# ttwang0303/Adaptive-RGBD-Localization-Mappig

Hardware: AMD Instinct MI355X
Metric: frames/sec (extract+match+RANSAC-PnP) @640x480, 2000 kp (higher is better)
Workload: dtype u8/i32 (extract, match), f32+f64 (ransac, pnp)

## Files before the change

### adaptive-rgbd-localization-mappig_amd/csrc/k_extract.hip

```cpp
#include "odo_device.h"
#include "odo_internal.h"
#ifdef FS_STATS
#include <cstdio>
#endif

#ifndef ODO_EXTRACT_PRIO
#define ODO_EXTRACT_PRIO 0
#endif
#define EXTRACT_PRIO() \
    if (ODO_EXTRACT_PRIO) __builtin_amdgcn_s_setprio(ODO_EXTRACT_PRIO)

namespace odo {

__global__ void __launch_bounds__(256) k_gray(const uint8_t* __restrict__ bgr, uint8_t* __restrict__ pyr,
                                              int w, int h, int pitch, size_t in_stride, size_t pyr_stride) {
    EXTRACT_PRIO();
    const int f = blockIdx.y;
    const int q = blockIdx.x * blockDim.x + threadIdx.x;
    const uint8_t* src = bgr + (size_t)f * in_stride;
    uint8_t* dst = pyr + (size_t)f * pyr_stride;
    const int npix = w * h;
    const int p0 = q * 4;
    if (p0 >= npix) return;
    const int y = p0 / w, x = p0 - y * w;
// ... 131 lines not shown
    const LevelDesc L = lv[G.level];
    const int R = G.rows, cols = G.cols, BW = G.bw, wcell = G.wcell, nc = G.ncell;
    constexpr int RS = FS_RS, RS4 = RS >> 2;
    const int sh = G.x0 & 15;
    {
        const uint4* src = reinterpret_cast<const uint4*>(pyr + (size_t)f * pyr_stride + L.off +
                                                          (size_t)G.y0 * L.pitch + (G.x0 & ~15));
        const int nw = (sh + cols + 15) >> 4, p16 = L.pitch >> 4;
        const int rstep = FS_TH / nw, k = t % nw, r0 = t / nw;
        if (r0 < rstep)
            for (int r = r0; r < R; r += rstep)
                reinterpret_cast<uint4*>(roi + r * RS)[k] = src[__umul24((uint32_t)r, (uint32_t)p16) + (uint32_t)k];
        for (int i = t; i < (R * RS) >> 4; i += FS_TH) reinterpret_cast<uint4*>(score)[i] = uint4{0, 0, 0, 0};
        for (int i = t; i < R * BW; i += FS_TH) bits[i] = 0;
        for (int i = t; i < R * FS_NCM; i += FS_TH) cnt[i] = 0;
        if (t == 0) M.ncl = 0, M.ovf = 0;
    }
    const int drows = R - 6;
    const int m0 = (sh + 3) >> 2, m1 = (sh + cols - 4) >> 2;
    {
        const uint32_t mlo = (0xFu << (sh + 3 - 4 * m0)) & 0xFu, mhi = (1u << (sh + cols - 3 - 4 * m1)) - 1u;
        if (t <= m1 - m0) {
            const int m = m0 + t;
            qlist[t] = uint2{fs_msb_mask((t == 0 ? mlo : 0xFu) & (m == m1 ? mhi : 0xFu)), 4u * (uint32_t)m};
        }
    }
    __syncthreads();
    const float inv_w = 1.0f / (float)wcell;
    uint32_t* const out = cand + ((size_t)f * ncells + G.ci0) * cell_cap;
    typedef short s16x2 __attribute__((ext_vector_type(2)));
    for (int pass = 0; pass < 2; pass++) {
        const int th = pass == 0 ? ini_th : min_th;
        const int thc = th < 0 ? 0 : (th > 255 ? 255 : th);
        const int NL = pass == 0 ? m1 - m0 + 1 : M.nl;
        const int items = drows > 0 && cols > 6 && NL > 0 ? drows * NL : 0;
        if (t == 0) FS_STAT(pass, items);
        {
            const s16x2 thv = {(short)thc, (short)thc};
            const float inl = NL > 0 ? 1.0f / (float)NL : 0.0f, inl_h = 0.5f * inl;
            int head = 0, tail = 0;
            auto seg_test = [&](int h, int n) {
                const int i0 = 2 * lane, i1 = i0 + 1;
                bool c0 = false, c1 = false;
                int o0 = 0, o1 = 0;
                if (i0 < n) {
                    o0 = ring[(h + i0) & (FS_RING - 1)];
                    o1 = i1 < n ? ring[(h + i1) & (FS_RING - 1)] : o0;
                    const s16x2 vv = {(short)roi[o0], (short)roi[o1]};
                    int a0 = o0 - 3 * RS - 3, a1 = o1 - 3 * RS - 3;
                    asm("" : "+v"(a0), "+v"(a1));
                    const uint8_t* const q0 = roi + a0;
                    const uint8_t* const q1 = roi + a1;
                    s16x2 d[16];
#pragma unroll
                    for (int k = 0; k < 16; k++) {
                        const int off = (kCircleDy[k] + 3) * RS + kCircleDx[k] + 3;
                        s16x2 c;
                        c.x = (short)q0[off];
                        c.y = (short)q1[off];
                        d[k] = vv - c;
                    }
                    s16x2 mn2[8], mx2[8], mn4[8], mx4[8];
#pragma unroll
                    for (int q = 0; q < 8; q++) {
                        const int j = 2 * q + 1;
                        mn2[q] = __builtin_elementwise_min(d[j], d[(j + 1) & 15]);
                        mx2[q] = __builtin_elementwise_max(d[j], d[(j + 1) & 15]);
                    }
#pragma unroll
                    for (int q = 0; q < 8; q++) {
                        mn4[q] = __builtin_elementwise_min(mn2[q], mn2[(q + 1) & 7]);
                        mx4[q] = __builtin_elementwise_max(mx2[q], mx2[(q + 1) & 7]);
                    }
                    s16x2 dk = s16x2{-32768, -32768}, br = s16x2{32767, 32767};
#pragma unroll
                    for (int q = 0; q < 8; q++) {
                        const int k = 2 * q;
                        const s16x2 m8 = __builtin_elementwise_min(mn4[q], mn4[(q + 2) & 7]);
                        const s16x2 x8 = __builtin_elementwise_max(mx4[q], mx4[(q + 2) & 7]);
                        dk = __builtin_elementwise_max(
                            dk, __builtin_elementwise_min(m8, __builtin_elementwise_max(d[k], d[(k + 9) & 15])));
                        br = __builtin_elementwise_min(
                            br, __builtin_elementwise_max(x8, __builtin_elementwise_min(d[k], d[(k + 9) & 15])));
                    }
                    const s16x2 sc = __builtin_elementwise_max(dk, -br);
                    c0 = sc.x > thc;
                    c1 = i1 < n && sc.y > thc;
                    if (c0) score[o0] = (uint8_t)(sc.x - 1);
                    if (c1) score[o1] = (uint8_t)(sc.y - 1);
                }
                const uint64_t b0 = __ballot(c0), b1 = __ballot(c1);
                const int nco = __popcll(b0) + __popcll(b1);
                if (lane == 0) FS_STAT(3, 1);
                if (nco) {
                    int cb = 0;
                    if (lane == 0) cb = atomicAdd(&M.ncl, nco);
                    cb = __shfl(cb, 0);
                    const int pre = (int)__builtin_amdgcn_mbcnt_hi((uint32_t)(b0 >> 32), __builtin_amdgcn_mbcnt_lo((uint32_t)b0, 0)) +
                                    (int)__builtin_amdgcn_mbcnt_hi((uint32_t)(b1 >> 32), __builtin_amdgcn_mbcnt_lo((uint32_t)b1, 0));
                    const int p0 = cb + pre, p1 = p0 + (c0 ? 1 : 0);
                    if (c0) { if (p0 < FS_CL) clist[p0] = (uint16_t)o0; else M.ovf = 1; }
                    if (c1) { if (p1 < FS_CL) clist[p1] = (uint16_t)o1; else M.ovf = 1; }
                }
            };
            for (int base = wave * 64; base < items; base += FS_TH) {
                uint32_t pass4 = 0;
                int qoff = 0;
                const int it = base + lane;
                if (it < items) {
                    const int ii = (int)__builtin_fmaf((float)it, inl, inl_h);
                    const int kk = it - __mul24(ii, NL);
                    const uint2 e = qlist[kk];
                    int wb = (int)__umul24((uint32_t)ii, (uint32_t)RS) + (int)e.y;
                    asm("" : "+v"(wb));
                    qoff = wb + 3 * RS;
                    const uint32_t* w = reinterpret_cast<const uint32_t*>(roi + wb);
                    const uint32_t Cw = w[3 * RS4], Uw = w[0], Dw = w[6 * RS4];
                    const uint32_t Lw = __builtin_amdgcn_alignbyte(Cw, w[3 * RS4 - 1], 1);
                    const uint32_t Rw = __builtin_amdgcn_alignbyte(w[3 * RS4 + 1], Cw, 3);
                    uint32_t hm[2];
#pragma unroll
                    for (int hh = 0; hh < 2; hh++) {
                        const uint32_t sel = hh ? 0x0c030c02u : 0x0c010c00u;
                        s16x2 v, a0, a4, a8, a12;
                        *reinterpret_cast<uint32_t*>(&v) = __builtin_amdgcn_perm(0u, Cw, sel);
                        *reinterpret_cast<uint32_t*>(&a0) = __builtin_amdgcn_perm(0u, Dw, sel);
                        *reinterpret_cast<uint32_t*>(&a4) = __builtin_amdgcn_perm(0u, Rw, sel);
                        *reinterpret_cast<uint32_t*>(&a8) = __builtin_amdgcn_perm(0u, Uw, sel);
                        *reinterpret_cast<uint32_t*>(&a12) = __builtin_amdgcn_perm(0u, Lw, sel);
                        const s16x2 dk = __builtin_elementwise_max(__builtin_elementwise_min(a0, a8),
                                                                   __builtin_elementwise_min(a4, a12));
                        const s16x2 bk = __builtin_elementwise_min(__builtin_elementwise_max(a0, a8),
                                                                   __builtin_elementwise_max(a4, a12));
                        const s16x2 t1 = dk - (v - thv), t2 = (v + thv) - bk;
                        hm[hh] = *reinterpret_cast<const uint32_t*>(&t1) | *reinterpret_cast<const uint32_t*>(&t2);
                    }
                    pass4 = __builtin_amdgcn_perm(hm[1], hm[0], 0x07050301u) & e.x;
                }
                uint32_t pos = (uint32_t)tail;
#pragma unroll
                for (int k = 0; k < 4; k++) {
                    const bool sv = (pass4 >> (8 * k + 7)) & 1u;
                    const uint64_t bk = __ballot(sv);
                    const uint32_t slot =
                        __builtin_amdgcn_mbcnt_hi((uint32_t)(bk >> 32), __builtin_amdgcn_mbcnt_lo((uint32_t)bk, pos)) &
                        (FS_RING - 1);
                    uint32_t at;
                    asm("v_cndmask_b32_e64 %0, %1, %2, %3" : "=v"(at) : "v"((uint32_t)FS_RING), "v"(slot), "s"(bk));
                    ring[at] = (uint16_t)(qoff + k);
                    pos += (uint32_t)__popcll(bk);
                }
                tail = (int)pos;
                if (tail - head >= 128) {
                    wave_lds_sync();
                    do {
                        seg_test(head, 128);
                        head += 128;
                    } while (tail - head >= 128);
                    wave_lds_sync();
                }
            }
            if (lane == 0) FS_STAT(2, tail);
            if (tail > head) {
                wave_lds_sync();
                seg_test(head, tail - head);
            }
        }
        __syncthreads();
        const bool ovf = M.ovf != 0;
        const int ncl = min(M.ncl, FS_CL);
        if (t == 0) FS_STAT(4, M.ncl), FS_STAT(5, ovf ? 1 : 0);
        auto locate = [&](int o, int& r, int& xs, int& jl, int& xl, int& xh) {
            r = o / RS;
            xs = (o - r * RS) - sh;
            jl = (int)(((float)(xs - 3) + 0.5f) * inv_w);
            xl = 3 + jl * wcell;
            xh = min(xl + wcell, cols - 3);
        };
        auto nms = [&](int o) {
            int so = o - RS - 1;
            asm("" : "+v"(so));
            const uint8_t* const sb = score + so;
            const int sc = sb[RS + 1];
            int r, xs, jl, xl, xh;
            locate(o, r, xs, jl, xl, xh);
            const int nmid = max((int)sb[1], (int)sb[2 * RS + 1]);
            const int nl = max(max((int)sb[0], (int)sb[RS]), (int)sb[2 * RS]);
            const int nr = max(max((int)sb[2], (int)sb[RS + 2]), (int)sb[2 * RS + 2]);
            const int nb = max(nmid, max(xs - 1 >= xl ? nl : 0, xs + 1 < xh ? nr : 0));
            if (sc > nb) {
                atomicOr(&bits[r * BW + (xs >> 5)], 1u << (xs & 31));
                atomicAdd(&cnt[r * FS_NCM + jl], 1);
            }
        };
        auto scan = [&](auto&& fn) {
            for (int it = t; it < items; it += FS_TH) {
                const int ii2 = it / NL, kk2 = it - ii2 * NL;
                const uint2 e = qlist[kk2];
                const uint32_t msk = e.x;
                const int qo = (3 + ii2) * RS + (int)e.y;
                for (int b = 0; b < 4; b++)
                    if (((msk >> (8 * b + 7)) & 1u) && score[qo + b]) fn(qo + b);
            }
        };
        if (!ovf)
            for (int i = t; i < ncl; i += FS_TH) nms(clist[i]);
        else
            scan(nms);
        __syncthreads();
        for (int j = wave; j < nc; j += FS_TH / 64) {
            if (pass == 1 && !M.retry[j]) continue;
            const int r = 3 + lane;
            const int v = lane < drows ? cnt[r * FS_NCM + j] : 0;
            int incl = v;
#pragma unroll
            for (int o = 1; o < 64; o <<= 1) {
                const int y = __shfl_up(incl, o);
                if (lane >= o) incl += y;
            }
            if (lane < drows) cnt[r * FS_NCM + j] = incl - v;
            if (lane == 63) M.tot[j] = incl;
        }
        __syncthreads();
        auto place = [&](int o) {
            int r, xs, jl, xl, xh;
            locate(o, r, xs, jl, xl, xh);
            const uint32_t* row = bits + r * BW;
            if (!((row[xs >> 5] >> (xs & 31)) & 1u)) return;
            int rank = cnt[r * FS_NCM + jl];
            const int wl = xl >> 5, nwd = (xs >> 5) - wl;
            const uint32_t hm = (1u << (xs & 31)) - 1u;
#pragma unroll
            for (int i = 0; i < 4; i++) {
                uint32_t v = row[wl + i];
                if (i == 0) v &= ~0u << (xl & 31);
                v &= i < nwd ? ~0u : (i == nwd ? hm : 0u);
                rank += __builtin_popcount(v);
            }
            if (rank < cell_cap)
                out[(size_t)jl * cell_cap + rank] = ((uint32_t)score[o] << 24) |
                                                    ((uint32_t)(r + G.y0 - 16) << 12) | (uint32_t)(xs + G.x0 - 16);
        };
        if (!ovf)
            for (int i = t; i < ncl; i += FS_TH) place(clist[i]);
        else
            scan(place);
        if (pass == 0) {
            if (t < nc) M.retry[t] = M.tot[t] == 0;
            __syncthreads();
            if (t < nc && M.retry[t]) FS_STAT(6, 1);
            if (t == 0) FS_STAT(7, nc);
            if (t < nc) {
                const int xa = sh + 3 + t * wcell, xe = sh + min(3 + (t + 1) * wcell, cols - 3);
                if (M.retry[t]) {
                    int at = 0;
                    for (int j = 0; j < t; j++)
                        if (M.retry[j]) {
                            const int ja = sh + 3 + j * wcell, je = sh + min(3 + (j + 1) * wcell, cols - 3);
                            at += ((je - 1) >> 2) - (ja >> 2) + 1;
                        }
                    for (int m = xa >> 2; m <= (xe - 1) >> 2; m++) {
                        const int lo = max(xa - 4 * m, 0), hi = min(xe - 4 * m, 4);
                        qlist[at++] = uint2{fs_msb_mask((0xFu << lo) & ((1u << hi) - 1u)), 4u * (uint32_t)m};
                    }
                } else {
                    cand_cnt[(size_t)f * ncells + G.ci0 + t] = min(M.tot[t], cell_cap);
                }
            }
            if (t == 0) {
                int n = 0;
                for (int j = 0; j < nc; j++)
                    if (M.retry[j]) {
                        const int ja = sh + 3 + j * wcell, je = sh + min(3 + (j + 1) * wcell, cols - 3);
                        n += ((je - 1) >> 2) - (ja >> 2) + 1;
                    }
                M.nl = n;
                M.ncl = 0;
                M.ovf = 0;
            }
            __syncthreads();
            if (M.nl == 0) return;
        } else if (t < nc && M.retry[t]) {
            cand_cnt[(size_t)f * ncells + G.ci0 + t] = min(M.tot[t], cell_cap);
        }
    }
}

struct ONode {
    int16_t x0, y0, x1, y1;
    int32_t cnt;
    int32_t seq;
};

#ifndef OT_THREADS
#define OT_THREADS 256
#endif

#ifndef OT_KB
#define OT_KB 8
#endif
#ifndef OT_RANK_MAX
#define OT_RANK_MAX 512
#endif
enum { OT_LDK = 1, OT_LDN = 2 };
template <bool RES, int LD, typename F>
ODO_INLINE void ot_pass(int n, int t, uint32_t (&rk)[OT_KB], int (&rn)[OT_KB], const uint32_t* keys, int32_t* knode,
                        F&& f) {
    if constexpr (RES) {
#pragma unroll
        for (int u = 0; u < OT_KB; u++)
            if (t + u * OT_THREADS < n) f(t + u * OT_THREADS, rk[u], rn[u]);
    } else {
        for (int k0 = t; k0 < n; k0 += OT_THREADS * OT_KB) {
#pragma unroll
            for (int u = 0; u < OT_KB; u++) {
                const int k = k0 + u * OT_THREADS;
                rn[u] = -1;
                if (k < n) {
                    if (LD & OT_LDK) rk[u] = keys[k];
                    if (LD & OT_LDN) rn[u] = knode[k];
                }
            }
#pragma unroll
            for (int u = 0; u < OT_KB; u++) {
                const int k = k0 + u * OT_THREADS;
                if (k < n) {
                    int node = rn[u];
                    f(k, rk[u], node);
                    if (node != rn[u]) knode[k] = node;
                }
            }
        }
    }
}

ODO_INLINE int block_exclusive_scan(int v, int* tmp, int* total);

ODO_INLINE int ot_gather(const uint32_t* __restrict__ cand, const int* __restrict__ cand_cnt, size_t cell0, int nc,
                         int cell_cap, uint32_t* dst, int cap, int* scan) {
    const int t = threadIdx.x;
    int n = 0;
    for (int cb = 0; cb < nc; cb += OT_THREADS) {
        const int c = cb + t;
        const int cnt = c < nc ? cand_cnt[cell0 + c] : 0;
        int tot;
        const int ex = block_exclusive_scan(cnt, scan, &tot);
        if (c < nc) {
            const uint4* src = reinterpret_cast<const uint4*>(cand + (cell0 + c) * cell_cap);
            uint32_t* d = dst + n + ex;
            const int room = cap - (n + ex);
            const int m = cnt < room ? cnt : room;
            for (int k0 = 0; k0 < m; k0 += 32) {
                uint4 v[8];
#pragma unroll
                for (int u = 0; u < 8; u++)
                    if (k0 + 4 * u < m) v[u] = src[(k0 >> 2) + u];
#pragma unroll
                for (int u = 0; u < 8; u++) {
                    const int k = k0 + 4 * u;
                    if (k < m) d[k] = v[u].x;
                    if (k + 1 < m) d[k + 1] = v[u].y;
                    if (k + 2 < m) d[k + 2] = v[u].z;
                    if (k + 3 < m) d[k + 3] = v[u].w;
                }
            }
        }
        n += tot;
    }
    return n;
}

ODO_INLINE uint64_t ot_key(int cnt, int seq, int pos) {
    return ((uint64_t)(uint32_t)cnt << 40) | ((uint64_t)(uint32_t)(seq & 0xFFFFFF) << 16) | (uint64_t)(pos & 0xFFFF);
}

ODO_INLINE int block_exclusive_scan(int v, int* tmp, int* total) {
    const int t = threadIdx.x, lane = t & 63, wave = t >> 6;
    const int x = wave_incl_scan(v);
    if (lane == 63) tmp[wave] = x;
    __syncthreads();
    int base = 0, tot = 0;
#pragma unroll
    for (int w = 0; w < OT_THREADS / 64; w++) {
        const int sw = tmp[w];
        if (w < wave) base += sw;
        tot += sw;
    }
    *total = tot;
    __syncthreads();
    return base + x - v;
}
ODO_INLINE int2 block_exclusive_scan2(int a, int b, int* tmp, int2* total) {
    constexpr int NWV = OT_THREADS / 64;
    const int t = threadIdx.x, lane = t & 63, wave = t >> 6;
    const int xa = wave_incl_scan(a), xb = wave_incl_scan(b);
    if (lane == 63) tmp[wave] = xa, tmp[NWV + wave] = xb;
    __syncthreads();
    int ba = 0, bb = 0, ta = 0, tb = 0;
#pragma unroll
    for (int w = 0; w < NWV; w++) {
        const int sa = tmp[w], sb = tmp[NWV + w];
        if (w < wave) ba += sa, bb += sb;
        ta += sa;
        tb += sb;
    }
    *total = int2{ta, tb};
    __syncthreads();
    return int2{ba + xa - a, bb + xb - b};
}

template <bool RES>
ODO_INLINE void ot_tree(const int n, const LevelDesc& L, char* smem, int* s_vars, const int node_cap,
                        uint32_t (&rk)[OT_KB], int (&rn)[OT_KB], const uint32_t* keys, int32_t* knode,
                        uint32_t* __restrict__ out, int* __restrict__ ocnt_fl, const int cap) {
    const int t = threadIdx.x;
    ONode* nodesA = reinterpret_cast<ONode*>(smem);
    ONode* nodesB = nodesA + node_cap;
    int* cc = reinterpret_cast<int*>(nodesB + node_cap);
    int* npos = cc + 4 * node_cap;
    int* iscr = npos + 4 * node_cap;
    int* scan = iscr + node_cap;
    uint64_t* sortk = reinterpret_cast<uint64_t*>(scan + OT_THREADS + 2);
    int& s_J = s_vars[6];
    int& s_size = s_vars[0];
    int& s_prev = s_vars[1];
    int& s_seq = s_vars[2];
    int& s_phase = s_vars[3];
    int& s_finish = s_vars[4];
    int& s_vcnt = s_vars[5];

    const int minX = 16, maxX = L.w - 16, minY = 16, maxY = L.h - 16;
    const int N = L.quota;
    const int nIni = (int)roundf((float)(maxX - minX) / (float)(maxY - minY));
    const float hX = (float)(maxX - minX) / (float)nIni;

    for (int i = t; i < nIni; i += OT_THREADS) {
        ONode nd;
        nd.x0 = (int16_t)(int)(hX * (float)i);
        nd.x1 = (int16_t)(int)(hX * (float)(i + 1));
        nd.y0 = 0;
        nd.y1 = (int16_t)(maxY - minY);
        nd.cnt = 0;
        nd.seq = i;
        nodesA[i] = nd;
    }
    __syncthreads();
    int ic0 = 0, ic1 = 0, ic2 = 0, ic3 = 0;
    ot_pass<RES, OT_LDK>(
        n, t, rk, rn, keys, knode, [&](int k, uint32_t key, int& node) {
            const float x = (float)(key & 0xfff);
            const int ni = (int)(x / hX);
            node = ni;
            ic0 += ni == 0;
            ic1 += ni == 1;
            ic2 += ni == 2;
            ic3 += ni == 3;
            if (ni > 3) atomicAdd(&nodesA[ni].cnt, 1);
        });
    if (ic0) atomicAdd(&nodesA[0].cnt, ic0);
    if (ic1) atomicAdd(&nodesA[1].cnt, ic1);
    if (ic2) atomicAdd(&nodesA[2].cnt, ic2);
    if (ic3) atomicAdd(&nodesA[3].cnt, ic3);
    __syncthreads();
    if (t == 0) {
        int w = 0;
        for (int i = 0; i < nIni; i++) {
            iscr[i] = -1;
            if (nodesA[i].cnt > 0) {
                iscr[i] = w;
                nodesB[w++] = nodesA[i];
            }
        }
        s_size = w;
        s_seq = nIni;
        s_finish = 0;
        s_phase = 1;
    }
    __syncthreads();
    ot_pass<RES, OT_LDN>(n, t, rk, rn, keys, knode, [&](int k, uint32_t key, int& node) { node = iscr[node]; });
    for (int i = t; i < s_size; i += OT_THREADS) nodesA[i] = nodesB[i];
    __syncthreads();

    ONode* cur = nodesA;
    ONode* nxt = nodesB;
    int vcount = 0;

    while (!s_finish) {
        const int S = s_size;
        if (s_phase == 1) {
            for (int i = t; i < 4 * S; i += OT_THREADS) cc[i] = 0;
            __syncthreads();
            ot_pass<RES, OT_LDK | OT_LDN>(
                n, t, rk, rn, keys, knode, [&](int k, uint32_t key, int& node) {
                    const ONode N0 = cur[node];
                    if (N0.cnt > 1) {
                        const int x = key & 0xfff, y = (key >> 12) & 0xfff;
                        const int hx = (N0.x1 - N0.x0 + 1) >> 1;
                        const int hy = (N0.y1 - N0.y0 + 1) >> 1;
                        const int q = (x < N0.x0 + hx) ? (y < N0.y0 + hy ? 0 : 2) : (y < N0.y0 + hy ? 1 : 3);
                        atomicAdd(&cc[node * 4 + q], 1);
                        node |= q << 16;
                    }
                });
            __syncthreads();
            int childBase = 0, survBase = 0, expBase = 0;
            int totalChildren = 0;
            for (int cb = 0; cb < S; cb += OT_THREADS) {
                const int i = cb + t;
                int e = 0, ne = 0, s = 0;
                if (i < S) {
                    if (cur[i].cnt > 1) {
#pragma unroll
                        for (int q = 0; q < 4; q++) {
                            e += cc[i * 4 + q] > 0;
                            ne += cc[i * 4 + q] > 1;
                        }
                    } else s = 1;
                }
                int2 tp;
                const int2 ex = block_exclusive_scan2(e | (ne << 16), s, scan, &tp);
                const int ex_e = ex.x & 0xFFFF, ex_ne = ex.x >> 16, ex_s = ex.y;
                const int te = tp.x & 0xFFFF, tne = tp.x >> 16, ts = tp.y;
                if (i < S) {
                    iscr[i] = childBase + ex_e;
                    npos[i * 4 + 0] = e;
                    npos[i * 4 + 1] = ex_ne + expBase;
                    npos[i * 4 + 2] = survBase + ex_s;
                    npos[i * 4 + 3] = s;
                }
                childBase += te;
                expBase += tne;
                survBase += ts;
                __syncthreads();
            }
            totalChildren = childBase;
            const int newSize = totalChildren + survBase;
            for (int i = t; i < S; i += OT_THREADS) {
                const ONode P = cur[i];
                const int e = npos[i * 4 + 0];
                const int vb = npos[i * 4 + 1];
                const int sr = npos[i * 4 + 2];
                if (npos[i * 4 + 3]) {
                    const int pos = totalChildren + sr;
                    nxt[pos] = P;
                    cc[i * 4 + 0] = pos;
                } else {
                    const int blockStart = totalChildren - (iscr[i] + e);
                    const int hx = (P.x1 - P.x0 + 1) >> 1, hy = (P.y1 - P.y0 + 1) >> 1;
                    int r = 0, v = vb;
                    int cpos[4];
#pragma unroll
                    for (int q = 0; q < 4; q++) {
                        const int c = cc[i * 4 + q];
                        cpos[q] = -1;
                        if (c > 0) {
                            ONode C;
                            const int qx = q & 1, qy = q >> 1;
                            C.x0 = (int16_t)(qx ? P.x0 + hx : P.x0);
                            C.x1 = (int16_t)(qx ? P.x1 : P.x0 + hx);
                            C.y0 = (int16_t)(qy ? P.y0 + hy : P.y0);
                            C.y1 = (int16_t)(qy ? P.y1 : P.y0 + hy);
                            C.cnt = c;
                            C.seq = s_seq + iscr[i] + r;
                            const int pos = blockStart + (e - 1 - r);
                            nxt[pos] = C;
                            cpos[q] = pos;
                            if (c > 1) {
                                sortk[v] = ot_key(c, C.seq, pos);
                                v++;
                            }
                            r++;
                        }
                    }
#pragma unroll
                    for (int q = 0; q < 4; q++) cc[i * 4 + q] = cpos[q];
                }
            }
            __syncthreads();
            ot_pass<RES, OT_LDN>(n, t, rk, rn, keys, knode, [&](int k, uint32_t key, int& node) {
                node = cc[(node & 0xFFFF) * 4 + (node >> 16)];
            });
            if (t == 0) {
                s_prev = S;
                s_size = newSize;
                s_seq += totalChildren;
                s_vcnt = expBase;
                if (newSize >= N || newSize == S) s_finish = 1;
                else if (newSize + expBase * 3 > N) s_phase = 2;
            }
            vcount = expBase;
            ONode* tmpp = cur;
            cur = nxt;
            nxt = tmpp;
        } else {
            vcount = s_vcnt;
            for (int i = t; i < S; i += OT_THREADS) iscr[i] = -1;
            if (vcount <= OT_RANK_MAX) {
                __syncthreads();
                for (int i = t; i < vcount; i += OT_THREADS) {
                    const uint64_t ki = sortk[i];
                    int above = 0, j = 0;
                    for (; j + 8 <= vcount; j += 8) {
                        uint64_t kj[8];
#pragma unroll
                        for (int u = 0; u < 8; u++) kj[u] = sortk[j + u];
#pragma unroll
                        for (int u = 0; u < 8; u++) above += kj[u] > ki;
                    }
                    for (; j < vcount; j++) above += sortk[j] > ki;
                    iscr[(int)(ki & 0xFFFF)] = above;
                }
                __syncthreads();
            } else {
                int pw = 1;
                while (pw < vcount) pw <<= 1;
                for (int i = vcount + t; i < pw; i += OT_THREADS) sortk[i] = ~0ull;
                __syncthreads();
                for (int kk = 2; kk <= pw; kk <<= 1) {
                    for (int jj = kk >> 1; jj > 0; jj >>= 1) {
                        for (int i = t; i < pw; i += OT_THREADS) {
                            const int ixj = i ^ jj;
                            if (ixj > i) {
                                const uint64_t a = sortk[i], b = sortk[ixj];
                                const bool up = (i & kk) == 0;
                                if ((a > b) == up) {
                                    sortk[i] = b;
                                    sortk[ixj] = a;
                                }
                            }
                        }
                        __syncthreads();
                    }
                }
                for (int j = t; j < vcount; j += OT_THREADS) iscr[(int)(sortk[vcount - 1 - j] & 0xFFFF)] = j;
                __syncthreads();
            }
            for (int i = t; i < 4 * S; i += OT_THREADS) cc[i] = 0;
            __syncthreads();
            ot_pass<RES, OT_LDK | OT_LDN>(
                n, t, rk, rn, keys, knode, [&](int k, uint32_t key, int& node) {
                    if (iscr[node] >= 0) {
                        const ONode N0 = cur[node];
                        const int x = key & 0xfff, y = (key >> 12) & 0xfff;
                        const int hx = (N0.x1 - N0.x0 + 1) >> 1;
                        const int hy = (N0.y1 - N0.y0 + 1) >> 1;
                        const int q = (x < N0.x0 + hx) ? (y < N0.y0 + hy ? 0 : 2) : (y < N0.y0 + hy ? 1 : 3);
                        atomicAdd(&cc[node * 4 + q], 1);
                        node |= q << 16;
                    }
                });
            __syncthreads();
            int* proc = npos;
            int* eincl = npos + node_cap;
            int* vexcl = npos + 2 * node_cap;
            for (int i = t; i < S; i += OT_THREADS)
                if (iscr[i] >= 0) proc[iscr[i]] = i;
            if (t == 0) s_J = vcount;
            __syncthreads();
            {
                int eb = 0, vb = 0;
                for (int cb = 0; cb < vcount; cb += OT_THREADS) {
                    const int j = cb + t;
                    int e = 0, v = 0;
                    if (j < vcount) {
                        const int i = proc[j];
#pragma unroll
                        for (int q = 0; q < 4; q++) {
                            e += cc[i * 4 + q] > 0;
                            v += cc[i * 4 + q] > 1;
                        }
                    }
                    int tot;
                    const int ex = block_exclusive_scan(e | (v << 16), scan, &tot);
                    if (j < vcount) {
                        const int ei = eb + (ex & 0xFFFF) + e;
                        eincl[j] = ei;
                        vexcl[j] = vb + (ex >> 16);
                        if (S + ei - (j + 1) >= N) atomicMin(&s_J, j + 1);
                    }
                    eb += tot & 0xFFFF;
                    vb += tot >> 16;
                }
            }
            __syncthreads();
            const int J = s_J;
            const int EJ = J > 0 ? eincl[J - 1] : 0;
            for (int j = t; j < J; j += OT_THREADS) {
                const int i = proc[j];
                const ONode P = cur[i];
                const int hx = (P.x1 - P.x0 + 1) >> 1, hy = (P.y1 - P.y0 + 1) >> 1;
                int e = 0;
#pragma unroll
                for (int q = 0; q < 4; q++) e += cc[i * 4 + q] > 0;
                const int blockStart = EJ - eincl[j];
                const int seqBase = s_seq + eincl[j] - e;
                int r = 0, v = vexcl[j];
                int cpos[4];
#pragma unroll
                for (int q = 0; q < 4; q++) {
                    const int c = cc[i * 4 + q];
                    cpos[q] = -1;
                    if (c > 0) {
                        ONode C;
                        const int qx = q & 1, qy = q >> 1;
                        C.x0 = (int16_t)(qx ? P.x0 + hx : P.x0);
                        C.x1 = (int16_t)(qx ? P.x1 : P.x0 + hx);
                        C.y0 = (int16_t)(qy ? P.y0 + hy : P.y0);
                        C.y1 = (int16_t)(qy ? P.y1 : P.y0 + hy);
                        C.cnt = c;
                        C.seq = seqBase + r;
                        const int pp = blockStart + (e - 1 - r);
                        nxt[pp] = C;
                        cpos[q] = pp;
                        if (c > 1) sortk[v++] = ot_key(c, C.seq, pp);
                        r++;
                    }
                }
#pragma unroll
                for (int q = 0; q < 4; q++) cc[i * 4 + q] = cpos[q];
                if (j == J - 1) s_vcnt = v;
            }
            int sb = 0;
            for (int cb = 0; cb < S; cb += OT_THREADS) {
                const int i = cb + t;
                int sv = 0;
                if (i < S) {
                    const int j = iscr[i];
                    sv = !(j >= 0 && j < J);
                }
                int tot;
                const int ex = block_exclusive_scan(sv, scan, &tot);
                if (sv) {
                    const int pp = EJ + sb + ex;
                    nxt[pp] = cur[i];
                    cc[i * 4 + 0] = pp;
                    iscr[i] = -2;
                }
                sb += tot;
            }
            if (t == 0) {
                const int size = EJ + sb;
                s_prev = S;
                s_size = size;
                s_seq += EJ;
                if (J == 0) s_vcnt = 0;
                if (size >= N || size == S) s_finish = 1;
            }
            __syncthreads();
            ot_pass<RES, OT_LDN>(n, t, rk, rn, keys, knode, [&](int k, uint32_t key, int& node) {
                const int i = node & 0xFFFF;
                node = cc[i * 4 + (iscr[i] < 0 ? 0 : node >> 16)];
            });
            ONode* tmpp = cur;
            cur = nxt;
            nxt = tmpp;
        }
        __syncthreads();
    }
    const int S = s_size;
    unsigned* best = reinterpret_cast<unsigned*>(cc);
    for (int i = t; i < S; i += OT_THREADS) best[i] = 0;
    __syncthreads();
    ot_pass<RES, OT_LDK | OT_LDN>(n, t, rk, rn, keys, knode, [&](int k, uint32_t key, int& node) {
        atomicMax(&best[node], ((key >> 24) << 23) | (0x7FFFFFu - (unsigned)k));
    });
    __syncthreads();
    ot_pass<RES, OT_LDK | OT_LDN>(n, t, rk, rn, keys, knode, [&](int k, uint32_t key, int& node) {
        if (node < cap && best[node] == (((key >> 24) << 23) | (0x7FFFFFu - (unsigned)k))) out[node] = key;
    });
    if (t == 0) *ocnt_fl = S < cap ? S : cap;
}

__global__ void __launch_bounds__(OT_THREADS) k_octree(const uint32_t* __restrict__ cand,
                                                       const int* __restrict__ cand_cnt, const LevelDesc* __restrict__ lv,
                                                       int ncells, int cell_cap, int nlevels,
                                                       uint32_t* __restrict__ keys_g, int32_t* __restrict__ knode_g,
                                                       size_t keys_stride_frame, uint32_t* __restrict__ okp,
                                                       int* __restrict__ ocnt, int okp_stride, int node_cap) {
    EXTRACT_PRIO();
    extern __shared__ __attribute__((aligned(16))) char smem[];
    __shared__ __attribute__((aligned(16))) int s_vars[16];
    const int f = blockIdx.y;
    const int l = (blockIdx.x + blockIdx.y) % nlevels;
    const int t = threadIdx.x;
    const LevelDesc L = lv[l];
    uint32_t* out = okp + ((size_t)f * nlevels + l) * okp_stride;
    int* ocnt_fl = ocnt + f * nlevels + l;
    const size_t cell0 = (size_t)f * ncells + L.cell_begin;
    const int nc = L.cell_end - L.cell_begin;
    int* scan = reinterpret_cast<int*>(smem) + 17 * node_cap;
    uint32_t* stage = reinterpret_cast<uint32_t*>(smem);
    const int res_cap = min(OT_THREADS * OT_KB, 16 * node_cap);
    uint32_t rk[OT_KB];
    int rn[OT_KB];

    const int n = ot_gather(cand, cand_cnt, cell0, nc, cell_cap, stage, res_cap, scan);
    __syncthreads();
    if (n == 0) {
        if (t == 0) *ocnt_fl = 0;
        return;
    }
    if (n <= res_cap) {
#pragma unroll
        for (int u = 0; u < OT_KB; u++)
            if (t + u * OT_THREADS < n) rk[u] = stage[t + u * OT_THREADS];
        __syncthreads();
        ot_tree<true>(n, L, smem, s_vars, node_cap, rk, rn, nullptr, nullptr, out, ocnt_fl, okp_stride);
    } else {
        const size_t kbase = (size_t)f * keys_stride_frame + (size_t)L.key_off;
        ot_gather(cand, cand_cnt, cell0, nc, cell_cap, keys_g + kbase, 0x7FFFFFFF, scan);
        __syncthreads();
        ot_tree<false>(n, L, smem, s_vars, node_cap, rk, rn, keys_g + kbase, knode_g + kbase, out, ocnt_fl,
                       okp_stride);
    }
}

#define BLUR_TX 128
#define BLUR_TY 32
#define BLUR_IW (BLUR_TX + 8)
#define BLUR_IH (BLUR_TY + 6)
ODO_INLINE int reflect101(int i, int n) {
    while (i < 0 || i >= n) i = i < 0 ? -i : 2 * n - 2 - i;
    return i;
}
ODO_INLINE int reflect101_1(int i, int n) { return i < 0 ? -i : (i >= n ? 2 * n - 2 - i : i); }

struct BlurTiles {
    int base[17];
    int tx[16];
};

typedef unsigned short blur_us2 __attribute__((ext_vector_type(2)));
ODO_INLINE uint32_t dot2u16(uint32_t a, uint32_t b, uint32_t c) {
    blur_us2 x, y;
    x.x = (unsigned short)(a & 0xffff), x.y = (unsigned short)(a >> 16);
    y.x = (unsigned short)(b & 0xffff), y.y = (unsigned short)(b >> 16);
    return __builtin_amdgcn_udot2(x, y, c, false);
}

__global__ void __launch_bounds__(256) k_blur(const uint8_t* __restrict__ pyr, uint8_t* __restrict__ blur,
                                              size_t pyr_stride, const LevelDesc* __restrict__ lv, BlurTiles TT,
                                              int nlevels) {
    __shared__ __attribute__((aligned(16))) uint8_t tile[BLUR_IH * BLUR_IW];
    __shared__ __attribute__((aligned(16))) uint32_t hrow[(BLUR_IH / 2) * BLUR_TX];
    const int f = blockIdx.y;
    const int tid = blockIdx.x;
    int l = 0;
    while (l + 1 < nlevels && tid >= TT.base[l + 1]) l++;
    const LevelDesc L = lv[l];
    const int ti = tid - TT.base[l];
    const int tx0 = (ti % TT.tx[l]) * BLUR_TX, ty0 = (ti / TT.tx[l]) * BLUR_TY;
    const uint8_t* src = pyr + (size_t)f * pyr_stride + L.off;
    uint8_t* dst = blur + (size_t)f * pyr_stride + L.off;
    const int t = threadIdx.x;
    const bool interior = tx0 >= 4 && ty0 >= 3 && tx0 + BLUR_TX + 4 <= L.w && ty0 + BLUR_TY + 3 <= L.h;
    if (interior) {
        constexpr int NW = BLUR_IW / 4;
        for (int it = t; it < BLUR_IH * NW; it += 256) {
            const int r = it / NW, c = it - r * NW;
            const uint32_t* srow = reinterpret_cast<const uint32_t*>(src + (size_t)(ty0 + r - 3) * L.pitch + tx0 - 4);
            reinterpret_cast<uint32_t*>(tile + r * BLUR_IW)[c] = srow[c];
        }
    } else {
        constexpr int NW = BLUR_IW / 4;
        for (int it = t; it < BLUR_IH * NW; it += 256) {
            const int r = it / NW, c = it - r * NW;
            const uint8_t* srow = src + (size_t)reflect101(ty0 + r - 3, L.h) * L.pitch;
            const int x = tx0 - 4 + 4 * c;
            uint32_t v;
            if (x >= 0 && x + 3 < L.w) {
                v = *reinterpret_cast<const uint32_t*>(srow + x);
            } else {
                v = 0;
#pragma unroll
                for (int b = 0; b < 4; b++) v |= (uint32_t)srow[reflect101(x + b, L.w)] << (8 * b);
            }
            reinterpret_cast<uint32_t*>(tile + r * BLUR_IW)[c] = v;
        }
    }
    __syncthreads();
    constexpr uint32_t C0 = 18u | (34u << 8) | (48u << 16) | (56u << 24);
    constexpr uint32_t C1 = 48u | (34u << 8) | (18u << 16);
    for (int it = t; it < (BLUR_IH / 2) * (BLUR_TX / 4); it += 256) {
        const int rp = it / (BLUR_TX / 4), q = it % (BLUR_TX / 4);
        uint32_t h[2][4];
#pragma unroll
        for (int e = 0; e < 2; e++) {
            const uint32_t* w = reinterpret_cast<const uint32_t*>(&tile[(2 * rp + e) * BLUR_IW + 4 * q]);
            const uint32_t w0 = w[0], w1 = w[1], w2 = w[2];
            h[e][0] = __builtin_amdgcn_udot4(__builtin_amdgcn_alignbyte(w2, w1, 1), C1,
                                             __builtin_amdgcn_udot4(__builtin_amdgcn_alignbyte(w1, w0, 1), C0, 0u, false),
                                             false);
            h[e][1] = __builtin_amdgcn_udot4(__builtin_amdgcn_alignbyte(w2, w1, 2), C1,
                                             __builtin_amdgcn_udot4(__builtin_amdgcn_alignbyte(w1, w0, 2), C0, 0u, false),
                                             false);
            h[e][2] = __builtin_amdgcn_udot4(__builtin_amdgcn_alignbyte(w2, w1, 3), C1,
                                             __builtin_amdgcn_udot4(__builtin_amdgcn_alignbyte(w1, w0, 3), C0, 0u, false),
                                             false);
            h[e][3] = __builtin_amdgcn_udot4(w2, C1, __builtin_amdgcn_udot4(w1, C0, 0u, false), false);
        }
        uint4 pk;
        pk.x = h[0][0] | (h[1][0] << 16);
        pk.y = h[0][1] | (h[1][1] << 16);
        pk.z = h[0][2] | (h[1][2] << 16);
        pk.w = h[0][3] | (h[1][3] << 16);
        *reinterpret_cast<uint4*>(&hrow[rp * BLUR_TX + 4 * q]) = pk;
    }
    __syncthreads();
    {
        const int q = t % (BLUR_TX / 4), rb = (t / (BLUR_TX / 4)) * 4;
        uint4 pk[5];
#pragma unroll
        for (int i = 0; i < 5; i++) pk[i] = *reinterpret_cast<const uint4*>(&hrow[(rb / 2 + i) * BLUR_TX + 4 * q]);
        constexpr uint32_t K01 = 18u | (34u << 16), K23 = 48u | (56u << 16), K45 = 48u | (34u << 16), K6 = 18u;
        uint32_t sum4[4][4];
#pragma unroll
        for (int cI = 0; cI < 4; cI++) {
            uint32_t E[5];
#pragma unroll
            for (int i = 0; i < 5; i++) E[i] = cI == 0 ? pk[i].x : cI == 1 ? pk[i].y : cI == 2 ? pk[i].z : pk[i].w;
            uint32_t P[10];
#pragma unroll
            for (int j = 0; j < 9; j++)
                P[j] = (j & 1) ? __builtin_amdgcn_perm(E[(j + 1) / 2], E[(j - 1) / 2], 0x05040302u) : E[j / 2];
            P[9] = E[4] >> 16;
#pragma unroll
            for (int o = 0; o < 4; o++) {
                uint32_t sum = dot2u16(P[o], K01, 32768u);
                sum = dot2u16(P[o + 2], K23, sum);
                sum = dot2u16(P[o + 4], K45, sum);
                sum4[o][cI] = dot2u16(P[o + 6], K6, sum);
            }
        }
        uint32_t out[4];
#pragma unroll
        for (int o = 0; o < 4; o++) {
            const uint32_t lo = __builtin_amdgcn_perm(sum4[o][1], sum4[o][0], 0x0c0c0602u);
            const uint32_t hi = __builtin_amdgcn_perm(sum4[o][3], sum4[o][2], 0x06020c0cu);
            out[o] = lo | hi;
        }
        const int x = tx0 + 4 * q;
        if (x < L.w) {
#pragma unroll
            for (int o = 0; o < 4; o++) {
                const int y = ty0 + rb + o;
                if (y < L.h) *reinterpret_cast<uint32_t*>(dst + (size_t)y * L.pitch + x) = out[o];
            }
        }
    }
}

#define BR_R 30
struct BlurRows {
    int base[17];
    int nst[16];
    int nq[16];
    int nch[16];
    int ebase[17];
};

ODO_INLINE uint32_t pair_lo(uint32_t cur, uint32_t prev) { return __builtin_amdgcn_perm(cur, prev, 0x05040100u); }
ODO_INLINE uint32_t pair_hi(uint32_t cur, uint32_t prev) { return __builtin_amdgcn_perm(cur, prev, 0x07060302u); }

template <int R>
ODO_INLINE int chunk_y0(int chunk, int h) { return min(chunk * R, h - R); }
#define BR_RE 6

template <bool EDGE, int R>
ODO_INLINE void blur_walk(const uint8_t* s0, uint8_t* dp, size_t pitch, int h, int y0, bool top, bool bottom,
                          bool store, int o0, int o1, int o2, const uint32_t (&selA)[3], const uint32_t (&selB)[3]) {
    constexpr uint32_t C0 = 18u | (34u << 8) | (48u << 16) | (56u << 24);
    constexpr uint32_t C1 = 48u | (34u << 8) | (18u << 16);
    constexpr uint32_t K01 = 18u | (34u << 16), K23 = 48u | (56u << 16), K45 = 48u | (34u << 16);
    constexpr uint32_t KLO = 18u, KHI = 18u << 16;
    uint32_t acc[6][4];
#pragma unroll
    for (int a = 0; a < 6; a++)
#pragma unroll
        for (int c = 0; c < 4; c++) acc[a][c] = 32768u;
    uint32_t hp0 = 0, hp1 = 0;
    static_assert(R % 6 == 0, "the accumulators rotate over 6 rows");
    constexpr int NB = (R + 6) / 6;
    uint32_t cw[6][3];
    const uint8_t* sp = s0 + (size_t)(y0 - 3) * pitch;
    auto load_row = [&](uint32_t(&d)[3], int b, int j, bool refl) {
        if (EDGE) {
            const uint8_t* rp = s0 + (size_t)reflect101_1(y0 - 3 + 6 * b + j, h) * pitch;
            d[0] = *reinterpret_cast<const uint32_t*>(rp + o0);
            d[1] = *reinterpret_cast<const uint32_t*>(rp + o1);
            d[2] = *reinterpret_cast<const uint32_t*>(rp + o2);
        } else {
            const uint8_t* rp = refl ? s0 + (size_t)reflect101_1(y0 - 3 + 6 * b + j, h) * pitch : sp + j * pitch;
            const uint32_t* w = reinterpret_cast<const uint32_t*>(rp);
            d[0] = w[0], d[1] = w[1], d[2] = w[2];
        }
    };
    auto load_block = [&](uint32_t(&d)[6][3], int b, bool refl) {
#pragma unroll
        for (int j = 0; j < 6; j++) load_row(d[j], b, j, refl);
        sp += 6 * pitch;
    };
    load_block(cw, 0, top);
    for (int b = 0; b < NB; b++) {
        const bool nref = b + 1 == NB - 1 && bottom;
#pragma unroll
        for (int j = 0; j < 6; j++) {
            uint32_t w0 = cw[j][0], w1 = cw[j][1], w2 = cw[j][2];
            if (b + 1 < NB) load_row(cw[j], b + 1, j, nref);
            if (EDGE) {
                const uint32_t e0 = __builtin_amdgcn_perm(w1, w0, selA[0]) | __builtin_amdgcn_perm(w2, w2, selB[0]);
                const uint32_t e1 = __builtin_amdgcn_perm(w1, w0, selA[1]) | __builtin_amdgcn_perm(w2, w2, selB[1]);
                const uint32_t e2 = __builtin_amdgcn_perm(w1, w0, selA[2]) | __builtin_amdgcn_perm(w2, w2, selB[2]);
                w0 = e0, w1 = e1, w2 = e2;
            }
            const uint32_t h0 = __builtin_amdgcn_udot4(__builtin_amdgcn_alignbyte(w2, w1, 1), C1,
                                                       __builtin_amdgcn_udot4(__builtin_amdgcn_alignbyte(w1, w0, 1), C0, 0u, false), false);
            const uint32_t h1 = __builtin_amdgcn_udot4(__builtin_amdgcn_alignbyte(w2, w1, 2), C1,
                                                       __builtin_amdgcn_udot4(__builtin_amdgcn_alignbyte(w1, w0, 2), C0, 0u, false), false);
            const uint32_t h2 = __builtin_amdgcn_udot4(__builtin_amdgcn_alignbyte(w2, w1, 3), C1,
                                                       __builtin_amdgcn_udot4(__builtin_amdgcn_alignbyte(w1, w0, 3), C0, 0u, false), false);
            const uint32_t h3 = __builtin_amdgcn_udot4(w2, C1, __builtin_amdgcn_udot4(w1, C0, 0u, false), false);
            const uint32_t hc0 = h0 | (h1 << 16), hc1 = h2 | (h3 << 16);
            const uint32_t P0 = pair_lo(hc0, hp0), P1 = pair_hi(hc0, hp0), P2 = pair_lo(hc1, hp1), P3 = pair_hi(hc1, hp1);
            hp0 = hc0;
            hp1 = hc1;
            const int sa = (j + 5) % 6, sb = (j + 3) % 6, sc = (j + 1) % 6, sd = j;
            acc[sa][0] = dot2u16(P0, K01, 32768u);
            acc[sa][1] = dot2u16(P1, K01, 32768u);
            acc[sa][2] = dot2u16(P2, K01, 32768u);
            acc[sa][3] = dot2u16(P3, K01, 32768u);
            acc[sb][0] = dot2u16(P0, K23, acc[sb][0]);
            acc[sb][1] = dot2u16(P1, K23, acc[sb][1]);
            acc[sb][2] = dot2u16(P2, K23, acc[sb][2]);
            acc[sb][3] = dot2u16(P3, K23, acc[sb][3]);
            acc[sc][0] = dot2u16(P0, K45, acc[sc][0]);
            acc[sc][1] = dot2u16(P1, K45, acc[sc][1]);
            acc[sc][2] = dot2u16(P2, K45, acc[sc][2]);
            acc[sc][3] = dot2u16(P3, K45, acc[sc][3]);
            const uint32_t s0v = dot2u16(hc0, KLO, acc[sd][0]), s1v = dot2u16(hc0, KHI, acc[sd][1]);
            const uint32_t s2v = dot2u16(hc1, KLO, acc[sd][2]), s3v = dot2u16(hc1, KHI, acc[sd][3]);
            if (b > 0 && store) {
                const uint32_t lo = __builtin_amdgcn_perm(s1v, s0v, 0x0c0c0602u);
                const uint32_t hi = __builtin_amdgcn_perm(s3v, s2v, 0x06020c0cu);
                *reinterpret_cast<uint32_t*>(dp) = lo | hi;
                dp += pitch;
            }
        }
        sp += 6 * pitch;
    }
}

ODO_INLINE void blur_edge_lane(const uint8_t* srcL, uint8_t* __restrict__ blur, size_t pyr_stride,
                                const LevelDesc* __restrict__ lv, const BlurRows& S, int nlevels, int f, int k) {
    if (k >= S.ebase[nlevels]) return;
    int l = 0;
    while (l + 1 < nlevels && k >= S.ebase[l + 1]) l++;
    const LevelDesc L = lv[l];
    const int nqa = (L.w + 3) >> 2, ne = 1 + nqa - (S.nq[l] + 1);
    const int i = k - S.ebase[l], chunk = i / ne, e = i - chunk * ne;
    const int q = e == 0 ? 0 : S.nq[l] + e;
    const int x = 4 * q;
    const int y0 = chunk_y0<BR_RE>(chunk, L.h);
    uint32_t selA[3], selB[3];
#pragma unroll
    for (int d = 0; d < 3; d++) {
        uint32_t a = 0, bsel = 0;
#pragma unroll
        for (int bb = 0; bb < 4; bb++) {
            const int src = reflect101_1(x - 4 + 4 * d + bb, L.w) - (x - 4);
            const int sd = src >> 2, sb = src & 3;
            a |= (uint32_t)(sd == 0 ? sb : sd == 1 ? 4 + sb : 0x0c) << (8 * bb);
            bsel |= (uint32_t)(sd == 2 ? sb : 0x0c) << (8 * bb);
        }
        selA[d] = a;
        selB[d] = bsel;
    }
    const int o0 = x >= 4 ? x - 4 : x, o2 = x + 8 <= L.pitch ? x + 4 : x;
    const uint8_t* s0 = srcL;
    uint8_t* dp = blur + (size_t)f * pyr_stride + L.off + (size_t)y0 * L.pitch + x;
    blur_walk<true, BR_RE>(s0, dp, (size_t)L.pitch, L.h, y0, true, true, true, o0, x, o2, selA, selB);
}

__global__ void __launch_bounds__(256) k_blur_rows(const uint8_t* __restrict__ pyr, uint8_t* __restrict__ blur,
                                                   size_t pyr_stride, const LevelDesc* __restrict__ lv, BlurRows S,
                                                   int nlevels, int eblocks) {
    EXTRACT_PRIO();
    const int f = blockIdx.y;
    if ((int)blockIdx.x < eblocks) {
        const int k = (int)blockIdx.x * 256 + (int)threadIdx.x;
        if (k >= S.ebase[nlevels]) return;
        int l = 0;
        while (l + 1 < nlevels && k >= S.ebase[l + 1]) l++;
        blur_edge_lane(pyr + (size_t)f * pyr_stride + lv[l].off, blur, pyr_stride, lv, S, nlevels, f, k);
        return;
    }
    const uint32_t none[3] = {0, 0, 0};
    const int item = ((int)blockIdx.x - eblocks) * 16 + ((int)threadIdx.x >> 4);
    if (item >= S.base[nlevels]) return;
    int l = 0;
    while (l + 1 < nlevels && item >= S.base[l + 1]) l++;
    const LevelDesc L = lv[l];
    const int it = item - S.base[l];
    const int chunk = it / S.nst[l], strip = it - chunk * S.nst[l];
    const int q = 1 + strip * 16 + ((int)threadIdx.x & 15);
    const bool store = q <= S.nq[l];
    const int x = 4 * (store ? q : S.nq[l]);
    const int y0 = chunk_y0<BR_R>(chunk, L.h);
    const bool top = y0 < 3, bottom = y0 + BR_R + 3 > L.h;
    const uint8_t* s0 = pyr + (size_t)f * pyr_stride + L.off + (x - 4);
    uint8_t* dp = blur + (size_t)f * pyr_stride + L.off + (size_t)y0 * L.pitch + x;
    blur_walk<false, BR_R>(s0, dp, (size_t)L.pitch, L.h, y0, top, bottom, store, 0, 0, 0, none, none);
}

#ifndef PYR_TH
#define PYR_TH 512
#endif
#ifndef PYR_VGPR
// ... 416 lines not shown
```

Before: 162,500.

## Precompute multi-level quadtree histogram to resolve early octree splits without per-level passes

Each keypoint's quadtree code is computed down to a depth D in a single pass, and per-cell counts are accumulated into a hierarchical histogram that is then reduced upward. The early subdivision levels are then built from that histogram without re-scanning keypoints each level, using a single wave while the node count stays within 64 and a block-wide loop otherwise. One final pass maps each keypoint's code to its node index. This aims to cut repeated full keypoint passes, atomics and block barriers in the first octree levels, at the cost of more shared-memory bookkeeping and added code complexity. Optional timestamp profiling behind a macro is also added.

```diff
diff --git a/adaptive-rgbd-localization-mappig_amd/csrc/k_extract.hip b/adaptive-rgbd-localization-mappig_amd/csrc/k_extract.hip
--- a/adaptive-rgbd-localization-mappig_amd/csrc/k_extract.hip
+++ b/adaptive-rgbd-localization-mappig_amd/csrc/k_extract.hip
@@ -457,6 +457,20 @@
 #ifndef OT_RANK_MAX
 #define OT_RANK_MAX 512
 #endif
+#ifdef ODO_OCTREE_PROFILE
+#define OT_NSTAMP 48
+__device__ unsigned long long g_ot_stamp[2][OT_NSTAMP];
+#define OT_STAMP(tag)                                                                                   \
+    do {                                                                                                \
+        if (threadIdx.x == 0 && s_vars[8] >= 0 && s_vars[8] < OT_NSTAMP)                                \
+            g_ot_stamp[s_vars[9]][s_vars[8]++] = ((unsigned long long)(tag) << 56) | (wall_clock64() & 0xFFFFFFFFFFFFFFull); \
+    } while (0)
+#else
+#define OT_STAMP(tag) ((void)0)
+#endif
+#ifndef OT_HIST_WAVE0
+#define OT_HIST_WAVE0 1
+#endif
 enum { OT_LDK = 1, OT_LDN = 2 };
 template <bool RES, int LD, typename F>
 ODO_INLINE void ot_pass(int n, int t, uint32_t (&rk)[OT_KB], int (&rn)[OT_KB], const uint32_t* keys, int32_t* knode,
@@ -589,55 +603,291 @@
     const int nIni = (int)roundf((float)(maxX - minX) / (float)(maxY - minY));
     const float hX = (float)(maxX - minX) / (float)nIni;
 
-    for (int i = t; i < nIni; i += OT_THREADS) {
-        ONode nd;
-        nd.x0 = (int16_t)(int)(hX * (float)i);
-        nd.x1 = (int16_t)(int)(hX * (float)(i + 1));
-        nd.y0 = 0;
-        nd.y1 = (int16_t)(maxY - minY);
-        nd.cnt = 0;
-        nd.seq = i;
-        nodesA[i] = nd;
-    }
+    if (nIni < 1) {
+        if (t == 0) *ocnt_fl = 0;
+        return;
+    }
+    int D = 0;
+    while (D < 4 && (nIni << (2 * D + 2)) <= node_cap) D++;
+    const int offD = nIni * ((1 << (2 * D)) - 1) / 3;
+    const int nT = offD + (nIni << (2 * D));
+    int* hist = cc;
+    int* postab = cc + nT;
+    uint16_t* tagA = reinterpret_cast<uint16_t*>(cc + 3 * node_cap);
+    uint16_t* tagB = tagA + node_cap;
+    for (int i = t; i < nT; i += OT_THREADS) hist[i] = 0;
     __syncthreads();
-    int ic0 = 0, ic1 = 0, ic2 = 0, ic3 = 0;
-    ot_pass<RES, OT_LDK>(
-        n, t, rk, rn, keys, knode, [&](int k, uint32_t key, int& node) {
-            const float x = (float)(key & 0xfff);
-            const int ni = (int)(x / hX);
-            node = ni;
-            ic0 += ni == 0;
-            ic1 += ni == 1;
-            ic2 += ni == 2;
-            ic3 += ni == 3;
-            if (ni > 3) atomicAdd(&nodesA[ni].cnt, 1);
-        });
-    if (ic0) atomicAdd(&nodesA[0].cnt, ic0);
-    if (ic1) atomicAdd(&nodesA[1].cnt, ic1);
-    if (ic2) atomicAdd(&nodesA[2].cnt, ic2);
-    if (ic3) atomicAdd(&nodesA[3].cnt, ic3);
+    ot_pass<RES, OT_LDK>(n, t, rk, rn, keys, knode, [&](int k, uint32_t key, int& node) {
+        const int x = key & 0xfff, y = (key >> 12) & 0xfff;
+        const int ni = min((int)((float)x / hX), nIni - 1);
+        int x0 = (int)(hX * (float)ni), x1 = (int)(hX * (float)(ni + 1)), y0 = 0, y1 = maxY - minY;
+        int code = ni;
+        for (int d = 0; d < D; d++) {
+            const int mx = x0 + ((x1 - x0 + 1) >> 1), my = y0 + ((y1 - y0 + 1) >> 1);
+            const bool right = x >= mx, low = y >= my;
+            x0 = right ? mx : x0;
+            x1 = right ? x1 : mx;
+            y0 = low ? my : y0;
+            y1 = low ? y1 : my;
+            code = code * 4 + (right ? 1 : 0) + (low ? 2 : 0);
+        }
+        atomicAdd(&hist[offD + code], 1);
+        node = code;
+    });
     __syncthreads();
-    if (t == 0) {
-        int w = 0;
-        for (int i = 0; i < nIni; i++) {
-            iscr[i] = -1;
-            if (nodesA[i].cnt > 0) {
-                iscr[i] = w;
-                nodesB[w++] = nodesA[i];
-            }
-        }
-        s_size = w;
-        s_seq = nIni;
-        s_finish = 0;
-        s_phase = 1;
+    OT_STAMP('H');
+    if (D > 0) {
+        const int w = nIni << (2 * D - 2), o = offD - w;
+        for (int j = t; j < w; j += OT_THREADS) {
+            const int* h = hist + offD + 4 * j;
+            hist[o + j] = h[0] + h[1] + h[2] + h[3];
+        }
     }
     __syncthreads();
-    ot_pass<RES, OT_LDN>(n, t, rk, rn, keys, knode, [&](int k, uint32_t key, int& node) { node = iscr[node]; });
-    for (int i = t; i < s_size; i += OT_THREADS) nodesA[i] = nodesB[i];
+    if (t < 64) {
+        int o1 = offD - (D > 0 ? nIni << (2 * D - 2) : 0);
+        for (int d = D - 2; d >= 0; d--) {
+            const int w = nIni << (2 * d), o = o1 - w;
+            for (int j = t; j < w; j += 64) {
+                const int* h = hist + o1 + 4 * j;
+                hist[o + j] = h[0] + h[1] + h[2] + h[3];
+            }
+            o1 = o;
+            wave_lds_sync();
+        }
+        if (t == 0) {
+            int w = 0;
+            for (int i = 0; i < nIni; i++) {
+                const int c = hist[i];
+                if (c > 0) {
+                    ONode nd;
+                    nd.x0 = (int16_t)(int)(hX * (float)i);
+                    nd.x1 = (int16_t)(int)(hX * (float)(i + 1));
+                    nd.y0 = 0;
+                    nd.y1 = (int16_t)(maxY - minY);
+                    nd.cnt = c;
+                    nd.seq = i;
+                    nodesA[w] = nd;
+                    tagA[w] = (uint16_t)i;
+                    w++;
+                }
+            }
+            s_size = w;
+            s_seq = nIni;
+            s_finish = 0;
+            s_phase = 1;
+        }
+    }
     __syncthreads();
+    OT_STAMP('I');
 
     ONode* cur = nodesA;
     ONode* nxt = nodesB;
+    {
+        uint16_t* ctag = tagA;
+        uint16_t* ntag = tagB;
+        int d = 0, od = 0;
+#if OT_HIST_WAVE0
+        if (t < 64) {
+            int S = s_size, seq = s_seq, prevS = S, vc = 0, fin = 0, ph = 1;
+            while (d < D && S <= 64) {
+                const int oc = od + (nIni << (2 * d));
+                ONode P0;
+                int tag = 0, e = 0, ne = 0, s = 0, hc[4] = {0, 0, 0, 0};
+                if (t < S) {
+                    P0 = cur[t];
+                    tag = ctag[t];
+                    if (P0.cnt > 1) {
+#pragma unroll
+                        for (int q = 0; q < 4; q++) {
+                            hc[q] = hist[oc + 4 * (tag - od) + q];
+                            e += hc[q] > 0;
+                            ne += hc[q] > 1;
+                        }
+                    } else s = 1;
+                }
+                const int v = e | (ne << 16);
+                const int xv = wave_incl_scan(v), xs = wave_incl_scan(s);
+                const int tv = __builtin_amdgcn_readlane(xv, 63), ts = __builtin_amdgcn_readlane(xs, 63);
+                const int totalChildren = tv & 0xFFFF, expBase = tv >> 16, newSize = totalChildren + ts;
+                const int ex_e = (xv - v) & 0xFFFF, ex_ne = (xv - v) >> 16, ex_s = xs - s;
+                if (t < S) {
+                    if (s) {
+                        const int pos = totalChildren + ex_s;
+                        nxt[pos] = P0;
+                        ntag[pos] = (uint16_t)tag;
+                    } else {
+                        const int blockStart = totalChildren - (ex_e + e);
+                        const int hx = (P0.x1 - P0.x0 + 1) >> 1, hy = (P0.y1 - P0.y0 + 1) >> 1;
+                        const int ctag0 = oc + 4 * (tag - od);
+                        int r = 0, vi = ex_ne;
+#pragma unroll
+                        for (int q = 0; q < 4; q++) {
+                            const int c = hc[q];
+                            if (c > 0) {
+                                ONode C;
+                                const int qx = q & 1, qy = q >> 1;
+                                C.x0 = (int16_t)(qx ? P0.x0 + hx : P0.x0);
+                                C.x1 = (int16_t)(qx ? P0.x1 : P0.x0 + hx);
+                                C.y0 = (int16_t)(qy ? P0.y0 + hy : P0.y0);
+                                C.y1 = (int16_t)(qy ? P0.y1 : P0.y0 + hy);
+                                C.cnt = c;
+                                C.seq = seq + ex_e + r;
+                                const int pos = blockStart + (e - 1 - r);
+                                nxt[pos] = C;
+                                ntag[pos] = (uint16_t)(ctag0 + q);
+                                if (c > 1) sortk[vi++] = ot_key(c, C.seq, pos);
+                                r++;
+                            }
+                        }
+                    }
+                }
+                prevS = S;
+                S = newSize;
+                seq += totalChildren;
+                vc = expBase;
+                ONode* tmpp = cur;
+                cur = nxt;
+                nxt = tmpp;
+                uint16_t* tmpt = ctag;
+                ctag = ntag;
+                ntag = tmpt;
+                od = oc;
+                d++;
+                wave_lds_sync();
+                OT_STAMP('1');
+                if (newSize >= N || newSize == prevS) fin = 1;
+                else if (newSize + expBase * 3 > N) ph = 2;
+                if (fin || ph == 2) break;
+            }
+            if (t == 0) {
+                if (d > 0) {
+                    s_prev = prevS;
+                    s_size = S;
+                    s_seq = seq;
+                    s_vcnt = vc;
+                    s_finish = fin;
+                    s_phase = ph;
+                }
+                s_J = d;
+            }
+        }
+        __syncthreads();
+        d = s_J;
+        od = nIni * ((1 << (2 * d)) - 1) / 3;
+        cur = (d & 1) ? nodesB : nodesA;
+        nxt = (d & 1) ? nodesA : nodesB;
+        ctag = (d & 1) ? tagB : tagA;
+        ntag = (d & 1) ? tagA : tagB;
+#endif
+        while (d < D && !s_finish && s_phase == 1) {
+            const int S = s_size, seq0 = s_seq;
+            const int oc = od + (nIni << (2 * d));
+            int childBase = 0, survBase = 0, expBase = 0;
+            for (int cb = 0; cb < S; cb += OT_THREADS) {
+                const int i = cb + t;
+                int e = 0, ne = 0, s = 0;
+                if (i < S) {
+                    if (cur[i].cnt > 1) {
+                        const int* h = hist + oc + 4 * (ctag[i] - od);
+#pragma unroll
+                        for (int q = 0; q < 4; q++) {
+                            e += h[q] > 0;
+                            ne += h[q] > 1;
+                        }
+                    } else s = 1;
+                }
+                int2 tp;
+                const int2 ex = block_exclusive_scan2(e | (ne << 16), s, scan, &tp);
+                if (i < S) {
+                    iscr[i] = childBase + (ex.x & 0xFFFF);
+                    npos[i * 4 + 0] = e;
+                    npos[i * 4 + 1] = (ex.x >> 16) + expBase;
+                    npos[i * 4 + 2] = survBase + ex.y;
+                    npos[i * 4 + 3] = s;
+                }
+                childBase += tp.x & 0xFFFF;
+                expBase += tp.x >> 16;
+                survBase += tp.y;
+            }
+            const int totalChildren = childBase;
+            const int newSize = totalChildren + survBase;
+            for (int i = t; i < S; i += OT_THREADS) {
+                const ONode P0 = cur[i];
+                const int tag = ctag[i];
+                const int e = npos[i * 4 + 0];
+                if (npos[i * 4 + 3]) {
+                    const int pos = totalChildren + npos[i * 4 + 2];
+                    nxt[pos] = P0;
+                    ntag[pos] = (uint16_t)tag;
+                } else {
+                    const int blockStart = totalChildren - (iscr[i] + e);
+                    const int hx = (P0.x1 - P0.x0 + 1) >> 1, hy = (P0.y1 - P0.y0 + 1) >> 1;
+                    const int ctag0 = oc + 4 * (tag - od);
+                    int r = 0, v = npos[i * 4 + 1];
+#pragma unroll
+                    for (int q = 0; q < 4; q++) {
+                        const int c = hist[ctag0 + q];
+                        if (c > 0) {
+                            ONode C;
+                            const int qx = q & 1, qy = q >> 1;
+                            C.x0 = (int16_t)(qx ? P0.x0 + hx : P0.x0);
+                            C.x1 = (int16_t)(qx ? P0.x1 : P0.x0 + hx);
+                            C.y0 = (int16_t)(qy ? P0.y0 + hy : P0.y0);
+                            C.y1 = (int16_t)(qy ? P0.y1 : P0.y0 + hy);
+                            C.cnt = c;
+                            C.seq = seq0 + iscr[i] + r;
+                            const int pos = blockStart + (e - 1 - r);
+                            nxt[pos] = C;
+                            ntag[pos] = (uint16_t)(ctag0 + q);
+                            if (c > 1) {
+                                sortk[v] = ot_key(c, C.seq, pos);
+                                v++;
+                            }
+                            r++;
+                        }
+                    }
+                }
+            }
+            if (t == 0) {
+                s_prev = S;
+                s_size = newSize;
+                s_seq = seq0 + totalChildren;
+                s_vcnt = expBase;
+                if (newSize >= N || newSize == S) s_finish = 1;
+                else if (newSize + expBase * 3 > N) s_phase = 2;
+            }
+            ONode* tmpp = cur;
+            cur = nxt;
+            nxt = tmpp;
+            uint16_t* tmpt = ctag;
+            ctag = ntag;
+            ntag = tmpt;
+            od = oc;
+            d++;
+            __syncthreads();
+            OT_STAMP('1');
+        }
+        const int S = s_size;
+        for (int i = t; i < S; i += OT_THREADS) postab[ctag[i]] = i;
+        __syncthreads();
+        ot_pass<RES, OT_LDN>(n, t, rk, rn, keys, knode, [&](int k, uint32_t key, int& node) {
+            const int code = node;
+            int idx[5], c[5], o = 0;
+#pragma unroll
+            for (int dd = 0; dd < 5; dd++) {
+                idx[dd] = o + (code >> (2 * max(D - dd, 0)));
+                o += nIni << (2 * dd);
+                c[dd] = dd < d ? hist[idx[dd]] : 1;
+            }
+            int sel = idx[4];
+#pragma unroll
+            for (int dd = 3; dd >= 0; dd--) sel = c[dd] == 1 ? idx[dd] : sel;
+            node = postab[sel];
+        });
+        __syncthreads();
+        OT_STAMP('L');
+    }
     int vcount = 0;
 
     while (!s_finish) {
@@ -744,6 +994,7 @@
                 else if (newSize + expBase * 3 > N) s_phase = 2;
             }
             vcount = expBase;
+            OT_STAMP('1');
             ONode* tmpp = cur;
             cur = nxt;
             nxt = tmpp;
@@ -906,6 +1157,7 @@
                 const int i = node & 0xFFFF;
                 node = cc[i * 4 + (iscr[i] < 0 ? 0 : node >> 16)];
             });
+            OT_STAMP('2');
             ONode* tmpp = cur;
             cur = nxt;
             nxt = tmpp;
@@ -924,6 +1176,7 @@
         if (node < cap && best[node] == (((key >> 24) << 23) | (0x7FFFFFu - (unsigned)k))) out[node] = key;
     });
     if (t == 0) *ocnt_fl = S < cap ? S : cap;
+    OT_STAMP('R');
 }
 
 __global__ void __launch_bounds__(OT_THREADS) k_octree(const uint32_t* __restrict__ cand,
@@ -948,9 +1201,17 @@
     const int res_cap = min(OT_THREADS * OT_KB, 16 * node_cap);
     uint32_t rk[OT_KB];
     int rn[OT_KB];
+#ifdef ODO_OCTREE_PROFILE
+    if (t == 0) {
+        s_vars[8] = f == 0 && (l == 0 || l == nlevels - 1) ? 0 : -1;
+        s_vars[9] = l != 0;
+    }
+    OT_STAMP('S');
+#endif
 
     const int n = ot_gather(cand, cand_cnt, cell0, nc, cell_cap, stage, res_cap, scan);
     __syncthreads();
+    OT_STAMP('G');
     if (n == 0) {
         if (t == 0) *ocnt_fl = 0;
         return;
@@ -968,6 +1229,14 @@
         ot_tree<false>(n, L, smem, s_vars, node_cap, rk, rn, keys_g + kbase, knode_g + kbase, out, ocnt_fl,
                        okp_stride);
     }
+#ifdef ODO_OCTREE_PROFILE
+    if (t == 0 && s_vars[8] > 0) {
+        const unsigned long long* st = g_ot_stamp[s_vars[9]];
+        for (int i = 1; i < s_vars[8]; i++)
+            printf("OTP level %d keys %d stamp %d %c %llu\n", l, n, i, (int)(st[i] >> 56),
+                   (st[i] - st[i - 1]) & 0xFFFFFFFFFFFFFFull);
+    }
+#endif
 }
 
 #define BLUR_TX 128
```

Measured after the change: 164,800, median of 6. +1.4%, better.
